# TUMFTM/CamRaDepth

Hardware: AMD Instinct MI355X
Metric: training images/sec at 256x416 bf16 (higher is better)
Workload: dtype bf16

## Files before the change

### camradepth_amd/csrc/encoder_ops.hip

```cpp
#include <stdlib.h>
#include "common.h"

namespace {

constexpr int TPB = 256;

constexpr int DTH = 8;
constexpr int DCW = 64;

struct InNorm {
  const crd_sum_t* stats;
  const float* gamma; const float* beta; int gmul;
};
__device__ __forceinline__ void innorm_coeffs(const InNorm& n, int b, int C, long long P, int c0, bool ok, float (&a)[8], float (&s)[8]) {
#pragma unroll
  for (int j = 0; j < 8; ++j) { a[j] = 1.f; s[j] = 0.f; }
  if (n.stats == nullptr || !ok) return;
  float mean, rstd;
  const int grp = (c0 >> 4) / n.gmul;
  gn_mean_rstd(n.stats + (long long)b * (C >> 4) * 2, grp * n.gmul, n.gmul, (float)P * 16.f * n.gmul, mean, rstd);
#pragma unroll
  for (int j = 0; j < 8; ++j) {
    a[j] = n.gamma[c0 + j] * rstd;
    s[j] = n.beta[c0 + j] - mean * a[j];
// ... 27 lines not shown
  const int b = blockIdx.z;
  const int c_win = blockIdx.y * DCW;
  const int tyi = blockIdx.x / tiles_x, txi = blockIdx.x - tyi * tiles_x;
  const int ty0 = tyi * DTH, tx0 = txi * TW;
  const bf16_t* xb = x + (long long)b * H * W * C;
  bf16_t* yb = y + (long long)b * H * W * C;
  const int t = threadIdx.x;
  const int nG = (C - c_win) >= DCW ? 8 : (C - c_win) >> 3;
  const int g = t & 7, xc = (t >> 3) % TW, rg = (t >> 3) / TW;
  const int c0 = c_win + g * 8;
  const bool gok = g < nG;
  typedef __attribute__((ext_vector_type(2))) float f32x2;
  f32x2 wv[9][4], bv[4];
  {
    uint4 r[(HPX * 8 + TPB - 1) / TPB];
    bool inimg[(HPX * 8 + TPB - 1) / TPB];
#pragma unroll
    for (int k = 0; k < (HPX * 8 + TPB - 1) / TPB; ++k) {
      const int i = t + k * TPB;
      const int hp = i >> 3, g = i & 7;
      const int hy = hp / HWD, hx = hp - hy * HWD;
      const int iy = ty0 - 1 + hy, ix = tx0 - 1 + hx;
      inimg[k] = i < HPX * 8 && g < nG && (unsigned)iy < (unsigned)H && (unsigned)ix < (unsigned)W;
      const int cy = iy < 0 ? 0 : (iy < H ? iy : H - 1), cx = ix < 0 ? 0 : (ix < W ? ix : W - 1), cgr = g < nG ? g : 0;
      const uint4 u = *reinterpret_cast<const uint4*>(xb + ((long long)cy * W + cx) * C + c_win + cgr * 8);
      r[k] = inimg[k] ? u : make_uint4(0, 0, 0, 0);
    }
#pragma unroll
    for (int tp = 0; tp < 9; ++tp) {
      float w8[8];
      if (gok) load8t<1>(w9, (long long)(FLIP ? 8 - tp : tp) * C + c0, w8);
      else {
#pragma unroll
        for (int j = 0; j < 8; ++j) w8[j] = 0.f;
      }
#pragma unroll
      for (int q = 0; q < 4; ++q) wv[tp][q] = f32x2{w8[2 * q], w8[2 * q + 1]};
    }
#pragma unroll
    for (int q = 0; q < 4; ++q) bv[q] = f32x2{(bias && gok) ? bias[c0 + 2 * q] : 0.f, (bias && gok) ? bias[c0 + 2 * q + 1] : 0.f};
    float na[8], ns[8];
    innorm_coeffs(inn, b, C, (long long)H * W, c_win + (t & 7) * 8, (t & 7) < nG, na, ns);
#pragma unroll
    for (int k = 0; k < (HPX * 8 + TPB - 1) / TPB; ++k) {
      const int i = t + k * TPB;
      if (i < HPX * 8) sh[i] = (inn.stats && inimg[k]) ? innorm_apply(r[k], na, ns) : r[k];
    }
  }
  uint4 xrv[ROWS];
  if (red.xr) {
    const int cgr = gok ? c0 : c_win;
#pragma unroll
    for (int i = 0; i < ROWS; ++i) {
      const int oy = ty0 + rg * ROWS + i, ox = tx0 + xc;
      const int cy = oy < H ? oy : H - 1, cx = ox < W ? ox : W - 1;
      xrv[i] = *reinterpret_cast<const uint4*>(red.xr + (((long long)b * H + cy) * W + cx) * C + cgr);
    }
  }
  __syncthreads();
  auto lds8 = [&](int hy, int hx, f32x2 (&v)[4]) {
    const uint4 u = sh[(hy * HWD + hx) * 8 + g];
    v[0] = f32x2{bf_lo(u.x), bf_hi(u.x)}; v[1] = f32x2{bf_lo(u.y), bf_hi(u.y)};
    v[2] = f32x2{bf_lo(u.z), bf_hi(u.z)}; v[3] = f32x2{bf_lo(u.w), bf_hi(u.w)};
  };
  f32x2 win[3][3][4];
  const int r0 = rg * ROWS;
#pragma unroll
  for (int ky = 0; ky < 2; ++ky)
#pragma unroll
    for (int kx = 0; kx < 3; ++kx) lds8(r0 + ky, xc + kx, win[ky][kx]);
  float s = 0.f, ss = 0.f;
  float rs0[8], rs1[8], rmean = 0.f, rrstd = 0.f;
#pragma unroll
  for (int j = 0; j < 8; ++j) rs0[j] = rs1[j] = 0.f;
  if (red.xr && gok) gn_mean_rstd(red.stats + (long long)b * (C >> 4) * 2, c0 >> 4, 1, (float)H * W * 16.f, rmean, rrstd);
#pragma unroll
  for (int i = 0; i < ROWS; ++i) {
#pragma unroll
    for (int kx = 0; kx < 3; ++kx) lds8(r0 + i + 2, xc + kx, win[(i + 2) % 3][kx]);
    const int oy = ty0 + r0 + i, ox = tx0 + xc;
    f32x2 acc[4];
#pragma unroll
    for (int q = 0; q < 4; ++q) acc[q] = bv[q];
#pragma unroll
    for (int ky = 0; ky < 3; ++ky)
#pragma unroll
      for (int kx = 0; kx < 3; ++kx) {
#pragma unroll
        for (int q = 0; q < 4; ++q) acc[q] = __builtin_elementwise_fma(win[(i + ky) % 3][kx][q], wv[ky * 3 + kx][q], acc[q]);
      }
    if (gok && oy < H && ox < W) {
      uint4 u;
      u.x = pack_bf2(acc[0][0], acc[0][1]); u.y = pack_bf2(acc[1][0], acc[1][1]); u.z = pack_bf2(acc[2][0], acc[2][1]); u.w = pack_bf2(acc[3][0], acc[3][1]);
      *reinterpret_cast<uint4*>(yb + ((long long)oy * W + ox) * C + c0) = u;
      if (red.xr) {
        const uint4 xv = xrv[i];
        const float gq[8] = {bf_lo(u.x), bf_hi(u.x), bf_lo(u.y), bf_hi(u.y), bf_lo(u.z), bf_hi(u.z), bf_lo(u.w), bf_hi(u.w)};
        const float xq[8] = {bf_lo(xv.x), bf_hi(xv.x), bf_lo(xv.y), bf_hi(xv.y), bf_lo(xv.z), bf_hi(xv.z), bf_lo(xv.w), bf_hi(xv.w)};
#pragma unroll
        for (int j = 0; j < 8; ++j) { rs0[j] += gq[j]; rs1[j] += gq[j] * ((xq[j] - rmean) * rrstd); }
      }
      if (STATS) {
        s += bf_lo(u.x) + bf_hi(u.x) + bf_lo(u.y) + bf_hi(u.y) + bf_lo(u.z) + bf_hi(u.z) + bf_lo(u.w) + bf_hi(u.w);
        ss += bf_lo(u.x) * bf_lo(u.x) + bf_hi(u.x) * bf_hi(u.x) + bf_lo(u.y) * bf_lo(u.y) + bf_hi(u.y) * bf_hi(u.y) +
              bf_lo(u.z) * bf_lo(u.z) + bf_hi(u.z) * bf_hi(u.z) + bf_lo(u.w) * bf_lo(u.w) + bf_hi(u.w) * bf_hi(u.w);
      }
    }
  }
  if (STATS) {
    s += __shfl_xor(s, 1); ss += __shfl_xor(ss, 1);
#pragma unroll
    for (int o = 8; o < 64; o <<= 1) { s += __shfl_xor(s, o); ss += __shfl_xor(ss, o); }
    const int wave = t >> 6, l = t & 63;
    if (l < 8 && (l & 1) == 0) { sred[wave][(l >> 1) * 2] = s; sred[wave][(l >> 1) * 2 + 1] = ss; }
    __syncthreads();
    if (t < 8) {
      const float v = sred[0][t] + sred[1][t] + sred[2][t] + sred[3][t];
      const int slab = (c_win >> 4) + (t >> 1);
      if (slab < (C >> 4)) stat_add(&stats[((long long)b * (C >> 4) + slab) * 2 + (t & 1)], v);
    }
  }
  if (red.xr) {
#pragma unroll
    for (int o = 8; o < 64; o <<= 1) {
#pragma unroll
      for (int j = 0; j < 8; ++j) { rs0[j] += __shfl_xor(rs0[j], o); rs1[j] += __shfl_xor(rs1[j], o); }
    }
    __syncthreads();
    float* fr = reinterpret_cast<float*>(sh);
    const int wave = t >> 6, l = t & 63;
    if (l < 8) {
#pragma unroll
      for (int j = 0; j < 8; ++j) { fr[wave * 128 + (l * 8 + j) * 2] = rs0[j]; fr[wave * 128 + (l * 8 + j) * 2 + 1] = rs1[j]; }
    }
    __syncthreads();
    const int nch = nG * 8;
    if (t < 2 * nch) {
      const float v = fr[t] + fr[128 + t] + fr[256 + t] + fr[384 + t];
      const int c = c_win + (t >> 1);
      grad_add(&red.r[((long long)b * C + c) * 2 + (t & 1)], v);
      fr[512 + t] = v * red.gamma[c];
    }
    __syncthreads();
    if (t < 2 * (nch >> 4)) {
      const int grp = t >> 1, which = t & 1;
      float a = 0.f;
#pragma unroll
      for (int j = 0; j < 16; ++j) a += fr[512 + (grp * 16 + j) * 2 + which];
      grad_add(&red.r[(long long)gridDim.z * C * 2 + ((long long)b * (C >> 4) + (c_win >> 4) + grp) * 2 + which], a);
    }
  }
}

#ifndef CRD_DWW_WGS
#define CRD_DWW_WGS 2
#endif
template <int TW>
__global__ __launch_bounds__(TPB, CRD_DWW_WGS) void k_dwconv_wgrad(const bf16_t* x, const bf16_t* dy, int H, int W, int C, crd_sum_t* dw10,
                                                      int replicas, int tiles_x, int tiles_y, int tiles_per_wg, InNorm inn) {
  constexpr int HWD = TW + 2;
  constexpr int HPX = (DTH + 2) * HWD;
  constexpr int RSPLIT = 32 / TW;
  constexpr int ROWS = DTH / RSPLIT;
  extern __shared__ __attribute__((aligned(16))) uint4 dsm[];
  uint4* sx = dsm;
  uint4* sdy = dsm + HPX * 8;
  const int b = blockIdx.z;
  const int c_win = blockIdx.y * DCW;
  const int txi = blockIdx.x % tiles_x, ygrp = blockIdx.x / tiles_x;
  const int tx0 = txi * TW;
  const bf16_t* xb = x + (long long)b * H * W * C;
  const bf16_t* db = dy + (long long)b * H * W * C;
  const int t = threadIdx.x;
  const int nG = (C - c_win) >= DCW ? 8 : (C - c_win) >> 3;
  const int g = t & 7, xc = (t >> 3) % TW, rg = (t >> 3) / TW;
  float acc[10][8];
#pragma unroll
  for (int tp = 0; tp < 10; ++tp)
#pragma unroll
    for (int j = 0; j < 8; ++j) acc[tp][j] = 0.f;
  auto unpack8 = [&](const uint4& u, float (&v)[8]) {
    v[0] = bf_lo(u.x); v[1] = bf_hi(u.x); v[2] = bf_lo(u.y); v[3] = bf_hi(u.y);
    v[4] = bf_lo(u.z); v[5] = bf_hi(u.z); v[6] = bf_lo(u.w); v[7] = bf_hi(u.w);
  };
  float na[8], ns[8];
  for (int it = 0; it < tiles_per_wg; ++it) {
    const int tyi = ygrp * tiles_per_wg + it;
    if (tyi >= tiles_y) break;
    const int ty0 = tyi * DTH;
    {
      constexpr int NX = (HPX * 8 + TPB - 1) / TPB, ND = (DTH * TW * 8) / TPB;
      uint4 rx[NX], rd[ND];
      bool inimg[NX];
#pragma unroll
      for (int k = 0; k < NX; ++k) {
        const int i = t + k * TPB;
        const int hp = i >> 3, gg = i & 7;
        const int hy = hp / HWD, hx = hp - hy * HWD;
        const int iy = ty0 - 1 + hy, ix = tx0 - 1 + hx;
        inimg[k] = i < HPX * 8 && gg < nG && (unsigned)iy < (unsigned)H && (unsigned)ix < (unsigned)W;
        const int cy = iy < 0 ? 0 : (iy < H ? iy : H - 1), cx = ix < 0 ? 0 : (ix < W ? ix : W - 1), cgr = gg < nG ? gg : 0;
        const uint4 u = *reinterpret_cast<const uint4*>(xb + ((long long)cy * W + cx) * C + c_win + cgr * 8);
        rx[k] = inimg[k] ? u : make_uint4(0, 0, 0, 0);
      }
#pragma unroll
      for (int k = 0; k < ND; ++k) {
        const int i = t + k * TPB;
        const int pp = i >> 3, gg = i & 7;
        const int py = pp / TW, px = pp - py * TW;
        const int iy = ty0 + py, ix = tx0 + px;
        const int cy = iy < H ? iy : H - 1, cx = ix < W ? ix : W - 1, cgr = gg < nG ? gg : 0;
        const uint4 u = *reinterpret_cast<const uint4*>(db + ((long long)cy * W + cx) * C + c_win + cgr * 8);
        rd[k] = (gg < nG && iy < H && ix < W) ? u : make_uint4(0, 0, 0, 0);
      }
      if (it == 0) innorm_coeffs(inn, b, C, (long long)H * W, c_win + (t & 7) * 8, (t & 7) < nG, na, ns);
      if (it > 0) __syncthreads();
#pragma unroll
      for (int k = 0; k < NX; ++k) {
        const int i = t + k * TPB;
        if (i < HPX * 8) sx[i] = (inn.stats && inimg[k]) ? innorm_apply(rx[k], na, ns) : rx[k];
      }
#pragma unroll
      for (int k = 0; k < ND; ++k) sdy[t + k * TPB] = rd[k];
    }
    __syncthreads();
    float win[3][3][8];
    const int r0 = rg * ROWS;
#pragma unroll
    for (int ky = 0; ky < 2; ++ky)
#pragma unroll
      for (int kx = 0; kx < 3; ++kx) unpack8(sx[((r0 + ky) * HWD + xc + kx) * 8 + g], win[ky][kx]);
#pragma unroll
    for (int i = 0; i < ROWS; ++i) {
#pragma unroll
      for (int kx = 0; kx < 3; ++kx) unpack8(sx[((r0 + i + 2) * HWD + xc + kx) * 8 + g], win[(i + 2) % 3][kx]);
      float d[8];
      unpack8(sdy[((r0 + i) * TW + xc) * 8 + g], d);
#pragma unroll
      for (int j = 0; j < 8; ++j) acc[9][j] += d[j];
#pragma unroll
      for (int ky = 0; ky < 3; ++ky)
#pragma unroll
        for (int kx = 0; kx < 3; ++kx) {
#pragma unroll
          for (int j = 0; j < 8; ++j) acc[ky * 3 + kx][j] += d[j] * win[(i + ky) % 3][kx][j];
        }
    }
  }
#pragma unroll
  for (int o = 8; o < 64; o <<= 1) {
#pragma unroll
    for (int tp = 0; tp < 10; ++tp)
#pragma unroll
      for (int j = 0; j < 8; ++j) acc[tp][j] += __shfl_xor(acc[tp][j], o);
  }
  __syncthreads();
  float* sm = reinterpret_cast<float*>(dsm);
  const int wave = t >> 6, l = t & 63;
  for (int w = 0; w < 4; ++w) {
    if (wave == w && l < 8) {
#pragma unroll
      for (int tp = 0; tp < 10; ++tp)
#pragma unroll
        for (int j = 0; j < 8; ++j) {
          float* p = &sm[tp * 64 + l * 8 + j];
          *p = w == 0 ? acc[tp][j] : *p + acc[tp][j];
        }
    }
    __syncthreads();
  }
  crd_sum_t* dst = dw10 + (long long)((blockIdx.z * gridDim.x + blockIdx.x) % replicas) * 10 * C;
  const int nch = nG * 8;
  for (int i = t; i < 10 * nch; i += TPB) {
    const int tp = i / nch, cl = i - tp * nch;
    const float v = sm[tp * 64 + cl];
    if (v != 0.f) grad_add(&dst[(long long)tp * C + c_win + cl], v);
  }
}

template <class PRE, class F>
__device__ __forceinline__ void matvec_rows(const bf16_t* w, int ld, int r_lo, int r_hi, int ncols, const float* sx, PRE&& pre, F&& out) {
  const int l = threadIdx.x & 63, wave = threadIdx.x >> 6, nw = blockDim.x >> 6;
  auto load_rows = [&](int r0, int c0, float (&wv)[4][8]) {
#pragma unroll
    for (int k = 0; k < 4; ++k) {
      const int r = r0 + k < r_hi ? r0 + k : r_hi - 1;
      load8(w + (long long)r * ld, c0 < ncols ? c0 : 0, 0, wv[k]);
    }
  };
  float w0[4][8];
  const int r_first = r_lo + wave * 4;
  load_rows(r_first < r_hi ? r_first : r_lo, l * 8, w0);
  pre();
  for (int r0 = r_first; r0 < r_hi; r0 += nw * 4) {
    double acc[4] = {0.0, 0.0, 0.0, 0.0};
    for (int c0 = l * 8; c0 < ncols; c0 += 512) {
      float wv[4][8];
      if (r0 == r_first && c0 == l * 8) {
#pragma unroll
        for (int k = 0; k < 4; ++k)
#pragma unroll
          for (int j = 0; j < 8; ++j) wv[k][j] = w0[k][j];
      } else {
        load_rows(r0, c0, wv);
      }
#pragma unroll
      for (int k = 0; k < 4; ++k)
#pragma unroll
        for (int j = 0; j < 8; ++j) acc[k] += (double)wv[k][j] * (double)sx[c0 + j];
    }
#pragma unroll
    for (int k = 0; k < 4; ++k)
#pragma unroll
      for (int o = 32; o > 0; o >>= 1) acc[k] += __shfl_xor(acc[k], o);
    if (l == 0) {
#pragma unroll
      for (int k = 0; k < 4; ++k)
        if (r0 + k < r_hi) out(r0 + k, (float)acc[k]);
    }
  }
}
constexpr int VEC_ROWS = 64;

struct XbarProj { const crd_sum_t* chan; const crd_sum_t* stats; const float* gamma; const float* beta; const bf16_t* w; int N, C; bf16_t* xbar; float* u; };
__device__ __forceinline__ void attn_xbar_proj_body(const XbarProj& x, int b, int e) {
  __shared__ float sx[1024];
  const int C = x.C, N = x.N, nt = blockDim.x;
  const int r_lo = e * VEC_ROWS, r_hi = r_lo + VEC_ROWS < C ? r_lo + VEC_ROWS : C;
  float* ub = x.u + (long long)b * C;
  matvec_rows(x.w, C, r_lo, r_hi, C, sx,
              [&]() {
                for (int c = threadIdx.x; c < C; c += nt) {
                  float mean, rstd;
                  gn_mean_rstd(x.stats + (long long)b * (C >> 4) * 2, c >> 4, 1, (float)N * 16.f, mean, rstd);
                  const float mc = stat_get(&x.chan[((long long)b * C + c) * 2]) / (float)N;
                  const bf16_t q = f2bf(x.gamma[c] * (mc - mean) * rstd + x.beta[c]);
                  if (e == 0) x.xbar[(long long)b * C + c] = q;
                  sx[c] = bf2f(q);
                }
                __syncthreads();
              },
              [&](int r, float v) { ub[r] = v; });
}

__global__ __launch_bounds__(1024) void k_attn_scores(const bf16_t* q, const bf16_t* k, int N, int M, int heads, int d,
                                                      float scale, float* S, short* idx, int qg, XbarProj xp) {
  __shared__ float smax[16][32];
  const int b = blockIdx.y;
  const int nvec = xp.chan ? (xp.C + VEC_ROWS - 1) / VEC_ROWS : 0;
  if ((int)blockIdx.x < nvec) { attn_xbar_proj_body(xp, b, blockIdx.x); return; }
  const int tile_x = blockIdx.x - nvec;
  const int l = threadIdx.x & 63, wave = threadIdx.x >> 6;
  const int h = wave % heads, g = wave / heads;
  const int n0 = (tile_x * qg + g) * 32;
  const int C = heads * d;
  const int n = n0 + (l & 31);
  const bool nok = n < N;
  const bf16_t* qb = q + ((long long)b * N + (nok ? n : 0)) * C;
  const bf16_t* kb = k + (long long)b * M * C;
  const int half = l >> 5;
  bf16x8 qf[4];
#pragma unroll
  for (int ks = 0; ks < 4; ++ks) {
    const int kk = ks * 16 + half * 8;
    uint4 u = *reinterpret_cast<const uint4*>(qb + h * d + (kk < d ? kk : 0));
    if (kk >= d) u = make_uint4(0, 0, 0, 0);
    qf[ks] = *reinterpret_cast<bf16x8*>(&u);
  }
  float best = -INFINITY;
  int besti = 0;
  const bool kcol_ok[4] = {half * 8 < d, 16 + half * 8 < d, 32 + half * 8 < d, 48 + half * 8 < d};
  auto load_keys = [&](int m0, uint4 (&dst)[4]) {
    int mrow = m0 + (l & 31);
    mrow = mrow < M ? mrow : M - 1;
    const bf16_t* rowp = kb + (long long)mrow * C + h * d;
#pragma unroll
    for (int ks = 0; ks < 4; ++ks) dst[ks] = *reinterpret_cast<const uint4*>(rowp + (kcol_ok[ks] ? ks * 16 + half * 8 : 0));
  };
  auto score_tile = [&](int m0, const uint4 (&kt)[4]) {
    f32x16 acc;
#pragma unroll
    for (int r = 0; r < 16; ++r) acc[r] = 0.f;
#pragma unroll
    for (int ks = 0; ks < 4; ++ks) {
      uint4 kf = kt[ks];
      if (!kcol_ok[ks]) kf = make_uint4(0, 0, 0, 0);
      acc = __builtin_amdgcn_mfma_f32_32x32x16_bf16(*reinterpret_cast<const bf16x8*>(&kf), qf[ks], acc, 0, 0, 0);
    }
    const bool edge = m0 + 32 > M;
#pragma unroll
    for (int r = 0; r < 16; r += 2) {
      const int ma = m0 + (r & 3) + 8 * (r >> 2) + 4 * half;
      const uint32_t p1 = pack_bf2(acc[r], acc[r + 1]);
      const uint32_t p2 = pack_bf2(bf_lo(p1) * scale, bf_hi(p1) * scale);
      float va = bf_lo(p2), vb = bf_hi(p2);
      if (edge) { va = ma < M ? va : -INFINITY; vb = ma + 1 < M ? vb : -INFINITY; }
      const bool ta = va > best;
      best = ta ? va : best;
      besti = ta ? ma : besti;
      const bool tb = vb > best;
      best = tb ? vb : best;
      besti = tb ? ma + 1 : besti;
    }
  };
  uint4 ring[4][4];
#pragma unroll
  for (int j = 0; j < 4; ++j) load_keys(j * 32, ring[j]);
  for (int m0 = 0; m0 < M; m0 += 128) {
#pragma unroll
    for (int j = 0; j < 4; ++j) {
      score_tile(m0 + j * 32, ring[j]);
      __builtin_amdgcn_sched_barrier(0);
      load_keys(m0 + j * 32 + 128, ring[j]);
      __builtin_amdgcn_sched_barrier(0);
    }
  }
  float ob = __shfl_xor(best, 32);
  int oi = __shfl_xor(besti, 32);
  if (ob > best || (ob == best && oi < besti)) { best = ob; besti = oi; }
  if (nok && half == 0) idx[((long long)b * N + n) * heads + h] = (short)besti;
  if (half == 0) smax[wave][l] = best;
  __syncthreads();
  if (h == 0 && half == 0 && nok) {
    float Ssum = 0.f;
    for (int hh = 0; hh < heads; ++hh) Ssum += smax[g * heads + hh][l];
    S[(long long)b * N + n] = Ssum;
  }
}
// ... 250 lines not shown
  const long long total = (long long)npx * CG;
  constexpr int UB = 4;
  for (long long i0 = threadIdx.x; i0 < total; i0 += (long long)UB * TPB) {
    int cgv[UB], mv[UB];
    long long nv[UB];
    float gv[UB];
#pragma unroll
    for (int u = 0; u < UB; ++u) {
      const long long i = i0 + (long long)u * TPB;
      const bool ok = i < total;
      cgv[u] = ok ? (int)(i % CG) : 0;
      nv[u] = ok ? p0 + i / CG : p0;
      const int h = (cgv[u] * 8) / d;
      mv[u] = idx[((long long)b * N + nv[u]) * heads + h];
      gv[u] = ok ? scale * dS[(long long)b * N + nv[u]] : 0.f;
    }
    uint4 kraw[UB], qraw[UB];
#pragma unroll
    for (int u = 0; u < UB; ++u) {
      kraw[u] = *reinterpret_cast<const uint4*>(k + ((long long)b * M + mv[u]) * C + cgv[u] * 8);
      qraw[u] = *reinterpret_cast<const uint4*>(q + ((long long)b * N + nv[u]) * C + cgv[u] * 8);
    }
#pragma unroll
    for (int u = 0; u < UB; ++u) {
      if (i0 + (long long)u * TPB >= total) continue;
      float kv[8];
      kv[0] = bf_lo(kraw[u].x); kv[1] = bf_hi(kraw[u].x); kv[2] = bf_lo(kraw[u].y); kv[3] = bf_hi(kraw[u].y);
      kv[4] = bf_lo(kraw[u].z); kv[5] = bf_hi(kraw[u].z); kv[6] = bf_lo(kraw[u].w); kv[7] = bf_hi(kraw[u].w);
#pragma unroll
      for (int j = 0; j < 8; ++j) kv[j] *= gv[u];
      store8_bf16(dq, ((long long)b * N + nv[u]) * C + cgv[u] * 8, kv);
      if (use_lds) {
        const int nl = (int)(nv[u] - p0);
        sq[nl * CG + cgv[u]] = qraw[u];
        const int h = (cgv[u] * 8) / d;
        if (cgv[u] * 8 == h * d) atomicOr(&mask[(h * M + mv[u]) * WPC + (nl >> 5)], 1u << (nl & 31));
        if (cgv[u] == 0) sg[nl] = gv[u];
      } else {
        float qv[8];
        qv[0] = bf_lo(qraw[u].x); qv[1] = bf_hi(qraw[u].x); qv[2] = bf_lo(qraw[u].y); qv[3] = bf_hi(qraw[u].y);
        qv[4] = bf_lo(qraw[u].z); qv[5] = bf_hi(qraw[u].z); qv[6] = bf_lo(qraw[u].w); qv[7] = bf_hi(qraw[u].w);
        crd_sum_t* dst = &dk[((long long)b * M + mv[u]) * C + cgv[u] * 8];
#pragma unroll
        for (int j = 0; j < 8; ++j) grad_add(dst + j, gv[u] * qv[j]);
      }
    }
  }
  if (!use_lds) return;
  __syncthreads();
  float* outp = dk_part ? dk_part + ((long long)chunk_x * gridDim.y + b) * M * C : nullptr;
  for (int pr = threadIdx.x; pr < M * CG; pr += TPB) {
    const int m = pr / CG, cg = pr - m * CG;
    const int h = (cg * 8) / d;
    const unsigned* mk = mask + (h * M + m) * WPC;
    float acc[8];
#pragma unroll
    for (int j = 0; j < 8; ++j) acc[j] = 0.f;
    for (int w = 0; w < WPC; ++w) {
      unsigned bits = mk[w];
      while (bits) {
        const int n = (w << 5) + __builtin_ctz(bits);
        bits &= bits - 1;
        const uint4 u = sq[n * CG + cg];
        const float g = sg[n];
        acc[0] += g * bf_lo(u.x); acc[1] += g * bf_hi(u.x); acc[2] += g * bf_lo(u.y); acc[3] += g * bf_hi(u.y);
        acc[4] += g * bf_lo(u.z); acc[5] += g * bf_hi(u.z); acc[6] += g * bf_lo(u.w); acc[7] += g * bf_hi(u.w);
      }
    }
    if (outp) {
      store8_f32(outp, (long long)m * C + cg * 8, acc);
    } else {
      crd_sum_t* dst = &dk[((long long)b * M + m) * C + cg * 8];
#pragma unroll
      for (int j = 0; j < 8; ++j)
        if (acc[j] != 0.f) grad_add(dst + j, acc[j]);
    }
  }
}

__global__ __launch_bounds__(TPB) void k_sum_partials_bf16(const float* part, int replicas, long long stride, bf16_t* dst, long long n8) {
  for (long long i = (long long)blockIdx.x * TPB + threadIdx.x; i < n8; i += (long long)gridDim.x * TPB) {
    float v[8];
#pragma unroll
    for (int j = 0; j < 8; ++j) v[j] = 0.f;
    for (int r0 = 0; r0 < replicas; r0 += 4) {
      float w[4][8];
#pragma unroll
      for (int k = 0; k < 4; ++k) load8(part, (long long)(r0 + k < replicas ? r0 + k : replicas - 1) * stride + i * 8, 1, w[k]);
#pragma unroll
      for (int k = 0; k < 4; ++k) {
        const bool ok = r0 + k < replicas;
#pragma unroll
        for (int j = 0; j < 8; ++j) v[j] += ok ? w[k][j] : 0.f;
      }
    }
    store8_bf16(dst, i * 8, v);
  }
}

__global__ __launch_bounds__(TPB) void k_gsum_to_bf16(const crd_sum_t* src, bf16_t* dst, long long n8) {
  for (long long i = (long long)blockIdx.x * TPB + threadIdx.x; i < n8; i += (long long)gridDim.x * TPB) {
    float v[8];
#pragma unroll
    for (int j = 0; j < 8; ++j) v[j] = grad_get(src + i * 8 + j);
    store8_bf16(dst, i * 8, v);
  }
}

}

static int dw_tile_width(int W) {
  static int forced = -1;
  if (forced < 0) forced = crd_dev_int("CRD_DW_TW", 0);
  if (forced == 16 || forced == 32) return forced;
  return W <= 16 ? 16 : 32;
}

extern "C" int crd_dwconv3x3(const void* x, int32_t B, int32_t H, int32_t W, int32_t C, const float* w9, const float* bias,
                             int32_t flip, void* y, crd_sum_t* stats, const crd_sum_t* in_stats, int32_t in_gmul,
                             const float* in_gamma, const float* in_beta, const void* red_x, const crd_sum_t* red_stats,
                             const float* red_gamma, crd_sum_t* red_r, crd_stream_t stream) {
  CRD_CHECK_ARG(x && w9 && y, "crd_dwconv3x3: null pointer");
  CRD_CHECK_ARG(!red_x || (red_stats && red_gamma && red_r), "crd_dwconv3x3: incomplete fused-reduce arguments");
  const RedOut red{reinterpret_cast<const bf16_t*>(red_x), red_stats, red_gamma, red_r};
  CRD_CHECK_ARG(!in_stats || (in_gamma && in_beta && in_gmul >= 1 && (C / 16) % in_gmul == 0), "crd_dwconv3x3: bad input-norm arguments");
  const InNorm inn{in_stats, in_gamma, in_beta, in_gmul};
  CRD_CHECK_ARG(C % 16 == 0, "crd_dwconv3x3: C must be a multiple of 16");
  const bf16_t* xp = reinterpret_cast<const bf16_t*>(x);
  bf16_t* yp = reinterpret_cast<bf16_t*>(y);
  hipStream_t st = as_stream(stream);
  const int tw = dw_tile_width(W);
  const int tiles_x = cdiv(W, tw), tiles_y = cdiv(H, DTH);
  dim3 grid(tiles_x * tiles_y, cdiv(C, DCW), B);
#define CRD_DW(FL, STT, TWV) hipLaunchKernelGGL((k_dwconv<FL, STT, TWV>), grid, dim3(TPB), 0, st, xp, H, W, C, w9, bias, yp, stats, tiles_x, inn, red)
  if (tw == 32) {
    if (flip) { if (stats) CRD_DW(true, true, 32); else CRD_DW(true, false, 32); }
    else { if (stats) CRD_DW(false, true, 32); else CRD_DW(false, false, 32); }
  } else {
    if (flip) { if (stats) CRD_DW(true, true, 16); else CRD_DW(true, false, 16); }
    else { if (stats) CRD_DW(false, true, 16); else CRD_DW(false, false, 16); }
  }
#undef CRD_DW
  CRD_LAUNCH_CHECK("crd_dwconv3x3");
  return CRD_OK;
}

extern "C" int crd_dwconv3x3_wgrad(const void* x, const void* dy, int32_t B, int32_t H, int32_t W, int32_t C, crd_sum_t* dw10,
                                   int32_t replicas, const crd_sum_t* in_stats, int32_t in_gmul, const float* in_gamma,
                                   const float* in_beta, crd_stream_t stream) {
  CRD_CHECK_ARG(x && dy && dw10 && replicas >= 1, "crd_dwconv3x3_wgrad: null pointer / replicas < 1");
  CRD_CHECK_ARG(!in_stats || (in_gamma && in_beta && in_gmul >= 1 && (C / 16) % in_gmul == 0), "crd_dwconv3x3_wgrad: bad input-norm arguments");
  const InNorm inn{in_stats, in_gamma, in_beta, in_gmul};
  CRD_CHECK_ARG(C % 16 == 0 && C <= 4096, "crd_dwconv3x3_wgrad: C must be a multiple of 16, <= 4096");
  const int tw = dw_tile_width(W);
  const int tiles_x = cdiv(W, tw), tiles_y = cdiv(H, DTH), wins = cdiv(C, DCW);
  int ysplit = cdiv(512, (long long)tiles_x * wins * B);
  if (ysplit > tiles_y) ysplit = tiles_y;
  if (ysplit < 1) ysplit = 1;
  const int per = cdiv(tiles_y, ysplit);
  ysplit = cdiv(tiles_y, per);
  dim3 grid(tiles_x * ysplit, wins, B);
  const bf16_t* xp = reinterpret_cast<const bf16_t*>(x);
  const bf16_t* dp = reinterpret_cast<const bf16_t*>(dy);
  hipStream_t st = as_stream(stream);
  static bool attr_done[2] = {false, false};
  if (tw == 32) {
    const size_t lds = (size_t)((DTH + 2) * 34 * 8 + DTH * 32 * 8) * sizeof(uint4);
    if (!attr_done[0]) { crd_reserve_lds(reinterpret_cast<const void*>(&k_dwconv_wgrad<32>), (int)lds, "k_dwconv_wgrad"); attr_done[0] = true; }
    hipLaunchKernelGGL(k_dwconv_wgrad<32>, grid, dim3(TPB), lds, st, xp, dp, H, W, C, dw10, replicas, tiles_x, tiles_y, per, inn);
  } else {
    const size_t lds = (size_t)((DTH + 2) * 18 * 8 + DTH * 16 * 8) * sizeof(uint4);
    if (!attr_done[1]) { crd_reserve_lds(reinterpret_cast<const void*>(&k_dwconv_wgrad<16>), (int)lds, "k_dwconv_wgrad"); attr_done[1] = true; }
    hipLaunchKernelGGL(k_dwconv_wgrad<16>, grid, dim3(TPB), lds, st, xp, dp, H, W, C, dw10, replicas, tiles_x, tiles_y, per, inn);
  }
  CRD_LAUNCH_CHECK("crd_dwconv3x3_wgrad");
  return CRD_OK;
}

static int attn_scores_launch(const void* q, const void* k, int32_t B, int32_t N, int32_t M, int32_t heads, int32_t d, float scale,
                              float* S, int16_t* idx, const XbarProj& xp, const char* who, crd_stream_t stream) {
  CRD_CHECK_ARG(q && k && S && idx, "%s: null pointer", who);
  CRD_UNSUPPORTED(d % 8 == 0 && d <= 64 && M < 32768, "%s: head dim must be a multiple of 8, <= 64 (got %d)", who, d);
  CRD_UNSUPPORTED(heads >= 1 && heads <= 16, "%s: at most 16 heads (got %d)", who, heads);
  int qg = 8 / heads;
  if (qg < 1) qg = 1;
  if (qg > 4) qg = 4;
  dim3 grid(cdiv(N, 32 * qg) + (xp.chan ? cdiv(xp.C, VEC_ROWS) : 0), B);
  hipLaunchKernelGGL(k_attn_scores, grid, dim3(64 * heads * qg), 0, as_stream(stream), reinterpret_cast<const bf16_t*>(q),
                     reinterpret_cast<const bf16_t*>(k), N, M, heads, d, scale, S, idx, qg, xp);
  CRD_LAUNCH_CHECK(who);
  return CRD_OK;
}

extern "C" int crd_attn_scores(const void* q, const void* k, int32_t B, int32_t N, int32_t M, int32_t heads, int32_t d,
                               float scale, float* S, int16_t* idx, crd_stream_t stream) {
  return attn_scores_launch(q, k, B, N, M, heads, d, scale, S, idx, XbarProj{}, "crd_attn_scores", stream);
}

extern "C" int crd_attn_scores_fp8(const void* q8, const void* k8, int32_t B, int32_t N, int32_t M, int32_t heads, float qk_scale,
                                   float scale, float* ssum, int16_t* idx, crd_stream_t stream) {
  CRD_CHECK_ARG(q8 && k8 && ssum && idx && B > 0 && N > 0 && M > 0 && qk_scale > 0.f, "crd_attn_scores_fp8: bad argument");
  CRD_UNSUPPORTED(heads >= 1 && heads <= 16, "crd_attn_scores_fp8: at most 16 heads");
  CRD_CHECK_ARG((reinterpret_cast<uintptr_t>(q8) & 15) == 0 && (reinterpret_cast<uintptr_t>(k8) & 15) == 0, "crd_attn_scores_fp8: 16-byte aligned operands");
  int qg = 8 / heads;
  if (qg < 1) qg = 1;
  if (qg > 4) qg = 4;
  hipLaunchKernelGGL(k_attn_scores_fp8, dim3(cdiv(N, 32 * qg), B), dim3(64 * heads * qg), 0, as_stream(stream),
                     reinterpret_cast<const unsigned char*>(q8), reinterpret_cast<const unsigned char*>(k8), N, M, heads, qk_scale, scale, ssum,
                     reinterpret_cast<short*>(idx), qg);
  CRD_LAUNCH_CHECK("crd_attn_scores_fp8");
  return CRD_OK;
}

extern "C" int crd_attn_fwd(const void* q, const void* k, int32_t B, int32_t N, int32_t M, int32_t heads, int32_t d, float scale,
                            float* S, int16_t* idx, const crd_sum_t* chan_sums, const crd_sum_t* stats, const float* gamma,
                            const float* beta, const void* w_fwd, void* xbar, float* u, crd_stream_t stream) {
  CRD_CHECK_ARG(chan_sums && stats && gamma && beta && w_fwd && xbar && u, "crd_attn_fwd: null pointer");
  const int C = heads * d;
  CRD_UNSUPPORTED(C % 16 == 0 && C <= 1024, "crd_attn_fwd: C must be a multiple of 16, <= 1024");
  return attn_scores_launch(q, k, B, N, M, heads, d, scale, S, idx,
                            XbarProj{chan_sums, stats, gamma, beta, reinterpret_cast<const bf16_t*>(w_fwd), N, C,
                                     reinterpret_cast<bf16_t*>(xbar), u}, "crd_attn_fwd", stream);
}

extern "C" int crd_attn_xbar(const crd_sum_t* chan_sums, const crd_sum_t* stats, const float* gamma, const float* beta, int32_t B,
                             int32_t N, int32_t C, void* xbar, crd_stream_t stream) {
  CRD_CHECK_ARG(chan_sums && stats && gamma && beta && xbar, "crd_attn_xbar: null pointer");
  hipLaunchKernelGGL(k_attn_xbar, dim3(B), dim3(256), 0, as_stream(stream), chan_sums, stats, gamma, beta, N, C,
                     reinterpret_cast<bf16_t*>(xbar));
  CRD_LAUNCH_CHECK("crd_attn_xbar");
  return CRD_OK;
}

extern "C" int crd_attn_xbar_proj(const crd_sum_t* chan_sums, const crd_sum_t* stats, const float* gamma, const float* beta, const void* w_fwd,
                                  int32_t B, int32_t N, int32_t C, void* xbar, float* u, crd_stream_t stream) {
  CRD_CHECK_ARG(chan_sums && stats && gamma && beta && w_fwd && xbar && u, "crd_attn_xbar_proj: null pointer");
  CRD_UNSUPPORTED(C % 16 == 0 && C <= 1024, "crd_attn_xbar_proj: C must be a multiple of 16, <= 1024");
  hipLaunchKernelGGL(k_attn_xbar_proj, dim3(cdiv(C, VEC_ROWS), B), dim3(TPB), 0, as_stream(stream),
                     XbarProj{chan_sums, stats, gamma, beta, reinterpret_cast<const bf16_t*>(w_fwd), N, C, reinterpret_cast<bf16_t*>(xbar), u});
  CRD_LAUNCH_CHECK("crd_attn_xbar_proj");
  return CRD_OK;
}

extern "C" int crd_attn_vec_bwd(const crd_sum_t* t, const void* w_dgrad, int32_t B, int32_t C, int32_t Cpad, float inv_n, void* tb, float* es,
                                crd_stream_t stream) {
  CRD_CHECK_ARG(t && w_dgrad && tb && es, "crd_attn_vec_bwd: null pointer");
  CRD_UNSUPPORTED(C % 8 == 0 && C <= 1024 && Cpad >= C && Cpad % 8 == 0, "crd_attn_vec_bwd: C must be a multiple of 8, <= 1024");
  hipLaunchKernelGGL(k_attn_vec_bwd, dim3(cdiv(C, VEC_ROWS), B), dim3(TPB), 0, as_stream(stream),
                     VecBwd{t, reinterpret_cast<const bf16_t*>(w_dgrad), C, Cpad, inv_n, reinterpret_cast<bf16_t*>(tb), es});
  CRD_LAUNCH_CHECK("crd_attn_vec_bwd");
  return CRD_OK;
}

extern "C" int crd_attn_out_residual(const float* x, const float* u, const float* S, const float* bp, const float* dp,
                                     int32_t B, int32_t N, int32_t C, float* x1, crd_stream_t stream) {
  CRD_CHECK_ARG(x && u && S && bp && x1, "crd_attn_out_residual: null pointer");
  CRD_CHECK_ARG(C % 8 == 0, "crd_attn_out_residual: C %% 8");
  const long long total = (long long)N * (C / 8);
  int nblk = cdiv(total, TPB);
  if (nblk > 2048) nblk = 2048;
  hipLaunchKernelGGL(k_attn_out_residual, dim3(nblk, B), dim3(TPB), 0, as_stream(stream), x, u, S, bp, dp, (long long)N, C, x1);
  CRD_LAUNCH_CHECK("crd_attn_out_residual");
  return CRD_OK;
}

static int attn_out_bwd_launch(float* dx1, const float* u, const float* S, const float* dp, int32_t B, int32_t N, int32_t C, crd_sum_t* t,
                               crd_sum_t* dbp_rows, float* dS, const GnPre* pre, const char* who, crd_stream_t stream) {
  CRD_CHECK_ARG(dx1 && u && S && t && dbp_rows && dS, "%s: null pointer", who);
  CRD_UNSUPPORTED(C % 8 == 0 && C <= 512, "%s: C must be a multiple of 8 and <= 512", who);
  static int small = -1;
  if (small < 0) small = crd_dev_int("CRD_ATTN_OUT_BWD_CHUNK", 32);
  int nblk = cdiv(N, (long long)B * cdiv(N, 256) < 128 ? small : 256);
  int cap = 1024 / (B > 0 ? B : 1); if (cap < 1) cap = 1;
  if (nblk > cap) nblk = cap;
  int chunk = cdiv(N, nblk);
  nblk = cdiv(N, chunk);
  if (pre) hipLaunchKernelGGL(k_attn_out_bwd<true>, dim3(nblk, B), dim3(TPB), 2 * C * sizeof(float), as_stream(stream), dx1, u, S, dp,
                              (long long)N, C, chunk, t, dbp_rows, dS, *pre);
  else hipLaunchKernelGGL(k_attn_out_bwd<false>, dim3(nblk, B), dim3(TPB), 2 * C * sizeof(float), as_stream(stream), dx1, u, S, dp,
                          (long long)N, C, chunk, t, dbp_rows, dS, GnPre{});
  CRD_LAUNCH_CHECK(who);
  return CRD_OK;
}

extern "C" int crd_attn_out_bwd(const float* dx1, const float* u, const float* S, const float* dp, int32_t B, int32_t N,
                                int32_t C, crd_sum_t* t, crd_sum_t* dbp_rows, float* dS, crd_stream_t stream) {
  return attn_out_bwd_launch(const_cast<float*>(dx1), u, S, dp, B, N, C, t, dbp_rows, dS, nullptr, "crd_attn_out_bwd", stream);
}

extern "C" int crd_attn_out_bwd_gn(float* dx1, const float* u, const float* S, const float* dp, int32_t B, int32_t N, int32_t C,
                                   crd_sum_t* t, crd_sum_t* dbp_rows, float* dS, const float* x, const void* dxn, const crd_sum_t* stats,
                                   const float* gamma, const crd_sum_t* r, float* dgamma, float* dbeta, crd_stream_t stream) {
  CRD_CHECK_ARG(x && dxn && stats && gamma && r, "crd_attn_out_bwd_gn: null pointer");
  CRD_CHECK_ARG(C % 16 == 0 && (dgamma == nullptr) == (dbeta == nullptr), "crd_attn_out_bwd_gn: C %% 16, dgamma / dbeta both or neither");
  const GnPre pre{x, reinterpret_cast<const bf16_t*>(dxn), stats, gamma, r, dgamma, dbeta, B};
  return attn_out_bwd_launch(dx1, u, S, dp, B, N, C, t, dbp_rows, dS, &pre, "crd_attn_out_bwd_gn", stream);
}

static size_t attn_bwd_lds(int chunk, int M, int heads, int C) {
  return (size_t)chunk * C * 2 + (size_t)chunk * 4 + (size_t)heads * M * ((chunk + 31) / 32) * 4 + 16;
}
static int attn_bwd_blocks(int B, int N, int M, int heads, int C) {
  static int small = -1, mid = -1;
  if (small < 0) {
    small = crd_dev_int("CRD_ATTN_BWD_CHUNK", 32);
    mid = crd_dev_int("CRD_ATTN_BWD_CHUNK2", 64);
  }
  int target = 128;
  if ((long long)B * cdiv(N, 128) < 128) target = N <= 512 ? small : mid;
  int nblk = cdiv(N, target);
  int cap = 2048 / (B > 0 ? B : 1); if (cap < 1) cap = 1;
  if (nblk > cap) nblk = cap;
  const int chunk = cdiv(N, nblk);
  if (attn_bwd_lds(chunk, M, heads, C) > 128 * 1024 || chunk > 32767) return 0;
  return cdiv(N, chunk);
}

extern "C" int crd_attn_scores_bwd_partials(int32_t B, int32_t N, int32_t M, int32_t heads, int32_t d) {
  return attn_bwd_blocks(B, N, M, heads, heads * d);
}

static int attn_scores_bwd_launch(const void* q, const void* k, const float* dS, const int16_t* idx, int32_t B, int32_t N,
                                  int32_t M, int32_t heads, int32_t d, float scale, void* dq, crd_sum_t* dk, float* dk_partials,
                                  const VecBwd& vec, const char* who, crd_stream_t stream) {
  CRD_CHECK_ARG(q && k && dS && idx && dq && (dk || dk_partials), "%s: null pointer", who);
  CRD_CHECK_ARG(d % 8 == 0, "%s: head dim must be a multiple of 8", who);
  const int C = heads * d;
// ... 62 lines not shown
```

Measured before the change: 455.7.

## Rewrite depthwise conv weight-grad as per-wave register-streamed column bands

Replaces the LDS-tiled depthwise 3x3 weight-gradient kernel with one where each wave owns a 4-column band over a run of rows. Each lane handles 2 channels and streams inputs through a rotating 3-row register window with software-prefetched global loads, so the shared-memory staging and its barriers go away. A persistent grid sized against a cost model picks the run length, and partial sums are reduced across 8 waves through LDS. The intended gain is less LDS traffic and synchronisation and better load/FMA overlap, at the price of narrow 4-byte per-lane loads and more register pressure.

```diff
diff --git a/camradepth_amd/csrc/encoder_ops.hip b/camradepth_amd/csrc/encoder_ops.hip
--- a/camradepth_amd/csrc/encoder_ops.hip
+++ b/camradepth_amd/csrc/encoder_ops.hip
@@ -203,128 +203,120 @@
   }
 }
 
-#ifndef CRD_DWW_WGS
-#define CRD_DWW_WGS 2
-#endif
-template <int TW>
-__global__ __launch_bounds__(TPB, CRD_DWW_WGS) void k_dwconv_wgrad(const bf16_t* x, const bf16_t* dy, int H, int W, int C, crd_sum_t* dw10,
-                                                      int replicas, int tiles_x, int tiles_y, int tiles_per_wg, InNorm inn) {
-  constexpr int HWD = TW + 2;
-  constexpr int HPX = (DTH + 2) * HWD;
-  constexpr int RSPLIT = 32 / TW;
-  constexpr int ROWS = DTH / RSPLIT;
-  extern __shared__ __attribute__((aligned(16))) uint4 dsm[];
-  uint4* sx = dsm;
-  uint4* sdy = dsm + HPX * 8;
-  const int b = blockIdx.z;
-  const int c_win = blockIdx.y * DCW;
-  const int txi = blockIdx.x % tiles_x, ygrp = blockIdx.x / tiles_x;
-  const int tx0 = txi * TW;
-  const bf16_t* xb = x + (long long)b * H * W * C;
-  const bf16_t* db = dy + (long long)b * H * W * C;
-  const int t = threadIdx.x;
-  const int nG = (C - c_win) >= DCW ? 8 : (C - c_win) >> 3;
-  const int g = t & 7, xc = (t >> 3) % TW, rg = (t >> 3) / TW;
-  float acc[10][8];
-#pragma unroll
-  for (int tp = 0; tp < 10; ++tp)
-#pragma unroll
-    for (int j = 0; j < 8; ++j) acc[tp][j] = 0.f;
-  auto unpack8 = [&](const uint4& u, float (&v)[8]) {
-    v[0] = bf_lo(u.x); v[1] = bf_hi(u.x); v[2] = bf_lo(u.y); v[3] = bf_hi(u.y);
-    v[4] = bf_lo(u.z); v[5] = bf_hi(u.z); v[6] = bf_lo(u.w); v[7] = bf_hi(u.w);
-  };
-  float na[8], ns[8];
-  for (int it = 0; it < tiles_per_wg; ++it) {
-    const int tyi = ygrp * tiles_per_wg + it;
-    if (tyi >= tiles_y) break;
-    const int ty0 = tyi * DTH;
-    {
-      constexpr int NX = (HPX * 8 + TPB - 1) / TPB, ND = (DTH * TW * 8) / TPB;
-      uint4 rx[NX], rd[ND];
-      bool inimg[NX];
-#pragma unroll
-      for (int k = 0; k < NX; ++k) {
-        const int i = t + k * TPB;
-        const int hp = i >> 3, gg = i & 7;
-        const int hy = hp / HWD, hx = hp - hy * HWD;
-        const int iy = ty0 - 1 + hy, ix = tx0 - 1 + hx;
-        inimg[k] = i < HPX * 8 && gg < nG && (unsigned)iy < (unsigned)H && (unsigned)ix < (unsigned)W;
-        const int cy = iy < 0 ? 0 : (iy < H ? iy : H - 1), cx = ix < 0 ? 0 : (ix < W ? ix : W - 1), cgr = gg < nG ? gg : 0;
-        const uint4 u = *reinterpret_cast<const uint4*>(xb + ((long long)cy * W + cx) * C + c_win + cgr * 8);
-        rx[k] = inimg[k] ? u : make_uint4(0, 0, 0, 0);
-      }
-#pragma unroll
-      for (int k = 0; k < ND; ++k) {
-        const int i = t + k * TPB;
-        const int pp = i >> 3, gg = i & 7;
-        const int py = pp / TW, px = pp - py * TW;
-        const int iy = ty0 + py, ix = tx0 + px;
-        const int cy = iy < H ? iy : H - 1, cx = ix < W ? ix : W - 1, cgr = gg < nG ? gg : 0;
-        const uint4 u = *reinterpret_cast<const uint4*>(db + ((long long)cy * W + cx) * C + c_win + cgr * 8);
-        rd[k] = (gg < nG && iy < H && ix < W) ? u : make_uint4(0, 0, 0, 0);
-      }
-      if (it == 0) innorm_coeffs(inn, b, C, (long long)H * W, c_win + (t & 7) * 8, (t & 7) < nG, na, ns);
-      if (it > 0) __syncthreads();
-#pragma unroll
-      for (int k = 0; k < NX; ++k) {
-        const int i = t + k * TPB;
-        if (i < HPX * 8) sx[i] = (inn.stats && inimg[k]) ? innorm_apply(rx[k], na, ns) : rx[k];
-      }
-#pragma unroll
-      for (int k = 0; k < ND; ++k) sdy[t + k * TPB] = rd[k];
-    }
-    __syncthreads();
-    float win[3][3][8];
-    const int r0 = rg * ROWS;
-#pragma unroll
-    for (int ky = 0; ky < 2; ++ky)
-#pragma unroll
-      for (int kx = 0; kx < 3; ++kx) unpack8(sx[((r0 + ky) * HWD + xc + kx) * 8 + g], win[ky][kx]);
-#pragma unroll
-    for (int i = 0; i < ROWS; ++i) {
-#pragma unroll
-      for (int kx = 0; kx < 3; ++kx) unpack8(sx[((r0 + i + 2) * HWD + xc + kx) * 8 + g], win[(i + 2) % 3][kx]);
-      float d[8];
-      unpack8(sdy[((r0 + i) * TW + xc) * 8 + g], d);
-#pragma unroll
-      for (int j = 0; j < 8; ++j) acc[9][j] += d[j];
-#pragma unroll
-      for (int ky = 0; ky < 3; ++ky)
-#pragma unroll
-        for (int kx = 0; kx < 3; ++kx) {
-#pragma unroll
-          for (int j = 0; j < 8; ++j) acc[ky * 3 + kx][j] += d[j] * win[(i + ky) % 3][kx][j];
+constexpr int DWW_CB = 4;
+constexpr int DWW_NW = 8;
+template <bool NRM>
+__global__ __launch_bounds__(64 * DWW_NW) void k_dwconv_wgrad(const bf16_t* x, const bf16_t* dy, int H, int W, int C, crd_sum_t* dw10,
+                                                              int replicas, int nbands, int rr, int nruns, int units, InNorm inn) {
+  typedef __attribute__((ext_vector_type(2))) float f32x2;
+  constexpr int XC = DWW_CB + 2;
+  extern __shared__ float fold[];
+  const int lane = threadIdx.x & 63, wave = __builtin_amdgcn_readfirstlane(threadIdx.x >> 6);
+  const int c_win = blockIdx.y * 128;
+  const int c = c_win + 2 * lane;
+  const bool cok = c < C;
+  f32x2 acc[10];
+#pragma unroll
+  for (int k = 0; k < 10; ++k) acc[k] = f32x2{0.f, 0.f};
+  for (int u = blockIdx.x * DWW_NW + wave; u < units; u += gridDim.x * DWW_NW) {
+    const int band = u % nbands, rest = u / nbands;
+    const int run = rest % nruns, b = rest / nruns;
+    const int x0 = band * DWW_CB, y0 = run * rr;
+    const char* xb = reinterpret_cast<const char*>(x + (long long)b * H * W * C);
+    const char* db = reinterpret_cast<const char*>(dy + (long long)b * H * W * C);
+    const unsigned loff = (cok ? c : 0) * 2;
+    auto at = [&](const char* base, int pix) { return *reinterpret_cast<const uint32_t*>(base + (long long)pix * C * 2 + loff); };
+    auto keep = [](bool ok) { uint32_t m = ok ? ~0u : 0u; asm volatile("" : "+v"(m)); return m; };
+    int xcol[XC];
+    bool xin[XC];
+#pragma unroll
+    for (int j = 0; j < XC; ++j) {
+      const int ix = x0 - 1 + j;
+      xin[j] = cok && (unsigned)ix < (unsigned)W;
+      xcol[j] = ix < 0 ? 0 : (ix < W ? ix : W - 1);
+    }
+    auto load_x = [&](int s, uint32_t (&r)[XC]) {
+      const int iy = y0 - 1 + s;
+      const bool rin = (unsigned)iy < (unsigned)H && s < rr + 2;
+      const int cy = iy < 0 ? 0 : (iy < H ? iy : H - 1);
+#pragma unroll
+      for (int j = 0; j < XC; ++j) {
+        r[j] = at(xb, cy * W + xcol[j]) & keep(rin && xin[j]);
+      }
+    };
+    auto load_d = [&](int i, uint32_t (&r)[DWW_CB]) {
+      const int iy = y0 + i;
+      const bool rin = iy < H && i < rr;
+      const int cy = iy < H ? iy : H - 1;
+#pragma unroll
+      for (int j = 0; j < DWW_CB; ++j) {
+        const int ix = x0 + j;
+        r[j] = at(db, cy * W + (ix < W ? ix : W - 1)) & keep(cok && rin && ix < W);
+      }
+    };
+    uint32_t rx[3][XC], rd[3][DWW_CB];
+    f32x2 xw[3][XC];
+    load_x(0, rx[0]); load_x(1, rx[1]); load_x(2, rx[2]);
+    load_d(0, rd[0]); load_d(1, rd[1]); load_d(2, rd[2]);
+    float na0 = 1.f, na1 = 1.f, ns0 = 0.f, ns1 = 0.f;
+    if (NRM && cok) {
+      float mean, rstd;
+      const int grp = (c >> 4) / inn.gmul;
+      gn_mean_rstd(inn.stats + (long long)b * (C >> 4) * 2, grp * inn.gmul, inn.gmul, (float)H * W * 16.f * inn.gmul, mean, rstd);
+      na0 = inn.gamma[c] * rstd; na1 = inn.gamma[c + 1] * rstd;
+      ns0 = inn.beta[c] - mean * na0; ns1 = inn.beta[c + 1] - mean * na1;
+    }
+    auto unpack_x = [&](int s, const uint32_t (&r)[XC], f32x2 (&v)[XC]) {
+      const bool rin = (unsigned)(y0 - 1 + s) < (unsigned)H;
+#pragma unroll
+      for (int j = 0; j < XC; ++j) {
+        uint32_t w = r[j];
+        if (NRM) {
+          const uint32_t wn = pack_bf2(bf_lo(w) * na0 + ns0, bf_hi(w) * na1 + ns1);
+          w = (rin && xin[j]) ? wn : 0u;
         }
-    }
-  }
-#pragma unroll
-  for (int o = 8; o < 64; o <<= 1) {
-#pragma unroll
-    for (int tp = 0; tp < 10; ++tp)
-#pragma unroll
-      for (int j = 0; j < 8; ++j) acc[tp][j] += __shfl_xor(acc[tp][j], o);
+        v[j] = f32x2{bf_lo(w), bf_hi(w)};
+      }
+    };
+    unpack_x(0, rx[0], xw[0]);
+    unpack_x(1, rx[1], xw[1]);
+    load_x(3, rx[0]); load_x(4, rx[1]);
+    for (int i0 = 0; i0 < rr; i0 += 3) {
+#pragma unroll
+      for (int k = 0; k < 3; ++k) {
+        const int i = i0 + k;
+        __builtin_amdgcn_sched_barrier(0);
+        unpack_x(i + 2, rx[(k + 2) % 3], xw[(k + 2) % 3]);
+        f32x2 d[DWW_CB];
+#pragma unroll
+        for (int j = 0; j < DWW_CB; ++j) d[j] = f32x2{bf_lo(rd[k][j]), bf_hi(rd[k][j])};
+        load_x(i + 5, rx[(k + 2) % 3]);
+        load_d(i + 3, rd[k]);
+#pragma unroll
+        for (int j = 0; j < DWW_CB; ++j) acc[9] += d[j];
+#pragma unroll
+        for (int ky = 0; ky < 3; ++ky)
+#pragma unroll
+          for (int kx = 0; kx < 3; ++kx)
+#pragma unroll
+            for (int j = 0; j < DWW_CB; ++j) acc[ky * 3 + kx] = __builtin_elementwise_fma(d[j], xw[(k + ky) % 3][j + kx], acc[ky * 3 + kx]);
+      }
+    }
+  }
+#pragma unroll
+  for (int k = 0; k < 10; ++k) {
+    fold[(wave * 20 + 2 * k) * 64 + lane] = acc[k][0];
+    fold[(wave * 20 + 2 * k + 1) * 64 + lane] = acc[k][1];
   }
   __syncthreads();
-  float* sm = reinterpret_cast<float*>(dsm);
-  const int wave = t >> 6, l = t & 63;
-  for (int w = 0; w < 4; ++w) {
-    if (wave == w && l < 8) {
-#pragma unroll
-      for (int tp = 0; tp < 10; ++tp)
-#pragma unroll
-        for (int j = 0; j < 8; ++j) {
-          float* p = &sm[tp * 64 + l * 8 + j];
-          *p = w == 0 ? acc[tp][j] : *p + acc[tp][j];
-        }
-    }
-    __syncthreads();
-  }
-  crd_sum_t* dst = dw10 + (long long)((blockIdx.z * gridDim.x + blockIdx.x) % replicas) * 10 * C;
-  const int nch = nG * 8;
-  for (int i = t; i < 10 * nch; i += TPB) {
-    const int tp = i / nch, cl = i - tp * nch;
-    const float v = sm[tp * 64 + cl];
+  crd_sum_t* dst = dw10 + (long long)(blockIdx.x % replicas) * 10 * C;
+  for (int i = threadIdx.x; i < 10 * 128; i += 64 * DWW_NW) {
+    const int tp = i >> 7, cl = i & 127;
+    if (c_win + cl >= C) continue;
+    const int row = 2 * tp + (cl & 1), l = cl >> 1;
+    float v = 0.f;
+#pragma unroll
+    for (int w = 0; w < DWW_NW; ++w) v += fold[(w * 20 + row) * 64 + l];
     if (v != 0.f) grad_add(&dst[(long long)tp * C + c_win + cl], v);
   }
 }
@@ -881,27 +873,32 @@
   CRD_CHECK_ARG(!in_stats || (in_gamma && in_beta && in_gmul >= 1 && (C / 16) % in_gmul == 0), "crd_dwconv3x3_wgrad: bad input-norm arguments");
   const InNorm inn{in_stats, in_gamma, in_beta, in_gmul};
   CRD_CHECK_ARG(C % 16 == 0 && C <= 4096, "crd_dwconv3x3_wgrad: C must be a multiple of 16, <= 4096");
-  const int tw = dw_tile_width(W);
-  const int tiles_x = cdiv(W, tw), tiles_y = cdiv(H, DTH), wins = cdiv(C, DCW);
-  int ysplit = cdiv(512, (long long)tiles_x * wins * B);
-  if (ysplit > tiles_y) ysplit = tiles_y;
-  if (ysplit < 1) ysplit = 1;
-  const int per = cdiv(tiles_y, ysplit);
-  ysplit = cdiv(tiles_y, per);
-  dim3 grid(tiles_x * ysplit, wins, B);
+  const int nbands = cdiv(W, DWW_CB), wins = cdiv(C, 128);
+  const long long cap = 256 / wins > 1 ? 256 / wins : 1;
+  int rr = 3;
+  long long best = -1;
+  for (int r = 3; r < H + 3; r += 3) {
+    const long long n = (long long)B * nbands * cdiv(H, r), per = cdiv(n, cap * DWW_NW);
+    const long long cost = per * (r + 6);
+    if (best < 0 || cost < best) { best = cost; rr = r; }
+  }
+  const int nruns = cdiv(H, rr);
+  const long long units = (long long)B * nbands * nruns;
+  CRD_UNSUPPORTED(units < (1ll << 30), "crd_dwconv3x3_wgrad: too many work units");
+  long long gx = cdiv(units, DWW_NW);
+  if (gx > cap) gx = cap;
+  dim3 grid((unsigned)gx, wins);
   const bf16_t* xp = reinterpret_cast<const bf16_t*>(x);
   const bf16_t* dp = reinterpret_cast<const bf16_t*>(dy);
-  hipStream_t st = as_stream(stream);
+  const int lds = DWW_NW * 20 * 64 * (int)sizeof(float);
   static bool attr_done[2] = {false, false};
-  if (tw == 32) {
-    const size_t lds = (size_t)((DTH + 2) * 34 * 8 + DTH * 32 * 8) * sizeof(uint4);
-    if (!attr_done[0]) { crd_reserve_lds(reinterpret_cast<const void*>(&k_dwconv_wgrad<32>), (int)lds, "k_dwconv_wgrad"); attr_done[0] = true; }
-    hipLaunchKernelGGL(k_dwconv_wgrad<32>, grid, dim3(TPB), lds, st, xp, dp, H, W, C, dw10, replicas, tiles_x, tiles_y, per, inn);
-  } else {
-    const size_t lds = (size_t)((DTH + 2) * 18 * 8 + DTH * 16 * 8) * sizeof(uint4);
-    if (!attr_done[1]) { crd_reserve_lds(reinterpret_cast<const void*>(&k_dwconv_wgrad<16>), (int)lds, "k_dwconv_wgrad"); attr_done[1] = true; }
-    hipLaunchKernelGGL(k_dwconv_wgrad<16>, grid, dim3(TPB), lds, st, xp, dp, H, W, C, dw10, replicas, tiles_x, tiles_y, per, inn);
-  }
+  const int nrm = inn.stats != nullptr;
+  const void* fn = nrm ? reinterpret_cast<const void*>(&k_dwconv_wgrad<true>) : reinterpret_cast<const void*>(&k_dwconv_wgrad<false>);
+  if (!attr_done[nrm]) { crd_reserve_lds(fn, lds, "k_dwconv_wgrad"); attr_done[nrm] = true; }
+  if (nrm) hipLaunchKernelGGL(k_dwconv_wgrad<true>, grid, dim3(64 * DWW_NW), lds, as_stream(stream), xp, dp, H, W, C, dw10, replicas, nbands, rr,
+                              nruns, (int)units, inn);
+  else hipLaunchKernelGGL(k_dwconv_wgrad<false>, grid, dim3(64 * DWW_NW), lds, as_stream(stream), xp, dp, H, W, C, dw10, replicas, nbands, rr,
+                          nruns, (int)units, inn);
   CRD_LAUNCH_CHECK("crd_dwconv3x3_wgrad");
   return CRD_OK;
 }
```

New measurement: 458.3, median of 6. No clear change (+0.6%).
